# DocF/multispectral-object-detection

Measured on AMD Instinct MI355X. Metric: image-pairs/sec fwd, yolov5l+CFTx3 640×640 bs64, 1/2/4/8 GPU, higher is better.
Workload: dtype bf16; 1 GPU; cfg3 (yolov5l_fusion_transformerx3_FLIR_aligned) two-stream forward, 640x640, 64 pairs/GPU, BN folded, pre-NMS detections; pairs_per_gpu=64, image_size=640, parallelism=batch-shard x1, hip_graph=True, two_hip_streams=False, forwards_in_flight=3, streams_per_forward_in_flight=1, single_in_flight_streams=2

## Files before the change

### include/cft_hip.h

```cpp
#ifndef CFT_HIP_H
#define CFT_HIP_H

#ifdef __cplusplus
extern "C" {
#endif

#define CFT_ABI_VERSION 19

enum { CFT_BF16 = 0, CFT_F32 = 1, CFT_F16 = 2 };
enum { CFT_ACT_NONE = 0, CFT_ACT_SILU = 1, CFT_ACT_GELU = 2 };
enum {
  CFT_OK = 0,
  CFT_EINVAL = -1,
  CFT_ELAUNCH = -2,
  CFT_ENODEV = -3
};

int cft_abi_version(void);
int cft_device_check(void);
const char* cft_last_error(void);
int cft_clock_probe(void* out4_u64, int spin_us, int* wall_khz, void* stream);

int cft_conv2d(const void* x, const void* w, const float* bias, const void* res, void* y,
               int B, int H, int W, int cin, int ldx, int xoff,
// ... 158 lines not shown

int cft_gpt_upsample_add2(const float* tokens, const void* base0, int ldb0, int boff0, const void* base1, int ldb1, int boff1,
                          void* out0, int ldo0, int ooff0, void* out1, int ldo1, int ooff1, void* sum, int lds, int soff,
                          int B, int H, int W, int C, int dtype, void* stream);

int cft_gpt_tokenize_grid(const void* rgb, int ld_rgb, int off_rgb, const void* ir, int ld_ir, int off_ir,
                          const float* pos_emb, float* tokens, int B, int H, int W, int C, int va, int ha,
                          int dtype, void* stream);

int cft_attention_tokens(const void* qkv, void* out, int B, int T, int heads, int dk, int dkp,
                         int dtype, float attn_pdrop, unsigned long long seed, void* stream);

int cft_gpt_upsample_add_grid(const float* tokens, int s, const void* base, int ldb, int boff,
                              void* out, int ldo, int ooff, int B, int H, int W, int C, int va, int ha,
                              int dtype, void* stream);

int cft_gpt_upsample_add2_grid(const float* tokens, const void* base0, int ldb0, int boff0, const void* base1, int ldb1, int boff1,
                               void* out0, int ldo0, int ooff0, void* out1, int ldo1, int ooff1, void* sum, int lds, int soff,
                               int B, int H, int W, int C, int va, int ha, int dtype, void* stream);

int cft_detect_decode(const float* logits, int ldl, float* raw, float* pred, const float* anchors,
                      int B, int ny, int nx, int na, int no, float stride,
                      long row0, long total_rows, void* stream);

long cft_batchnorm_train_workspace(long M, int C);
int cft_batchnorm_train(const float* x, int ldx, int xoff, long M, int C,
                        const float* gamma, const float* beta, float* running_mean, float* running_var,
                        float momentum, float eps, const void* res, int ldr, int roff, int res_dtype,
                        void* y, int ldy, int yoff, int act, int out_dtype,
                        void* workspace, long workspace_bytes, void* stream);
int cft_dropout(void* x, long n, float p, unsigned long long seed, int dtype, void* stream);

int cft_nms(const float* pred, int B, int rows, int no, float conf_thres, float iou_thres,
            int agnostic, int multi_label, const unsigned char* class_allow, int max_det, int max_nms,
            void* scratch, long scratch_bytes, float* dets, int* counts, void* stream);

long cft_eval_match_workspace_bytes(int B, int nt);
int cft_eval_match(const float* dets, const int* counts, int B, int max_det, const float* targets, int nt, int img_h, int img_w,
                   const float* geom, const float* iouv_host, int niou, int single_cls, void* workspace, long workspace_bytes,
                   unsigned char* correct, unsigned short* tp_bits, float* conf, int* pcls, int* label_hist, int nc,
                   int* tcls, int* nl, void* stream);

long cft_eval_ap_workspace_bytes(long n, int nc);
int cft_eval_ap(const unsigned short* tp_bits, const float* conf, const int* pcls, long n, int niou, const int* label_hist, int nc,
                const double* px, const double* x, void* workspace, long workspace_bytes, double* out, void* stream);

// ... 80 lines not shown
```

### multispectral-object-detection_amd/_lib.py

```python
import ctypes
import os
import re
import subprocess

import torch

_HERE = os.path.dirname(os.path.abspath(__file__))
LIB_PATH = os.environ.get("CFT_HIP_LIB") or os.path.join(_HERE, "libcft_hip.so")
CSRC = os.path.join(_HERE, "csrc")
SOURCES = ("runtime.hip", "conv_gemm.hip", "conv_gemm_asm.hip", "focus_conv.hip", "bottleneck.hip", "pointwise.hip", "attention.hip", "attention_tokens.hip", "nms.hip", "train.hip", "metrics.hip", "confusion.hip", "loss.hip", "autoanchor.hip", "dataset.hip", "detect.hip", "optim.hip", "mosaic.hip", "augment.hip", "jpeg.hip", "jpeg_encode.hip")

HEADER = os.path.join(_HERE, "..", "include", "cft_hip.h")
HEADERS = ("cft_common.h", "conv_common.h", "focus_common.h", "bneck_common.h", "metrics_common.h", "resize_common.h", "conv_gemm_asm.inc")

_SCALARS = {"int": ctypes.c_int, "long": ctypes.c_long, "float": ctypes.c_float, "unsigned long long": ctypes.c_ulonglong}
_RETURNS = {"int": ctypes.c_int, "long": ctypes.c_long, "const char*": ctypes.c_char_p}
_TYPE_WORDS = frozenset("void char short int long float double signed unsigned const".split())


def parse_header(text):
    text = re.sub(r"/\*.*?\*/|//[^\n]*", " ", text, flags=re.S)
    consts = {k: int(v) for k, v in re.findall(r"(?:#define\s+|\b)(CFT_\w+)\s*=?\s*(-?\d+)\b", text)}
    text = re.sub(r"^\s*#.*$", "", text, flags=re.M)
    sigs = {}
    for ret, name, args in re.findall(r"([\w\s*]+?)\b(cft_\w+)\s*\(([^()]*)\)\s*;", text):
        ret = re.sub(r"\s*\*", "*", " ".join(ret.split()))
        if ret not in _RETURNS:
            raise ValueError(f"{name}: unknown return type '{ret}'")
        argtypes = []
        for arg in ([] if args.strip() in ("", "void") else args.split(",")):
            *kind, pname = [w for w in arg.split() if w != "const"] or [""]
            if "*" in arg:
                argtypes.append(ctypes.c_void_p)
            elif " ".join(kind) in _SCALARS and pname not in _TYPE_WORDS:
                argtypes.append(_SCALARS[" ".join(kind)])
            else:
# ... 73 lines not shown
```

### multispectral-object-detection_amd/csrc/conv_common.h

```cpp
#pragma once
#include "cft_common.h"
#include <stdlib.h>

struct ConvParams {
  const unsigned char* x;
  const unsigned char* w;
  const float* bias;
  const unsigned char* res;
  unsigned char* y;
  int H, W, Cin, ldx, xoff;
  int Ho, Wo, N, Kpad, K;
  int ldy, yoff, ldr, roff;
  int KS, stride, pad;
  int act, out_f32, res_f32;
  int M, tilesN;
  const unsigned char* w2;
  const float* bias2;
  int N2;
  unsigned char* y1;
  int ldy1, yoff1;
  int ksplit, ksteps;
  long x_bytes, w_bytes;
  uint32_t wo_mul, wo_sh, ho_mul, ho_sh;
};

__device__ __forceinline__ int fast_div(int n, uint32_t mul, uint32_t sh) {
  return mul ? (int)(__umulhi((uint32_t)n, mul) >> sh) : n;
}

static __device__ __attribute__((aligned(16))) uint32_t cft_zero_page[4] = {0u, 0u, 0u, 0u};
constexpr int CFT_ZERO_REGION_BYTES = 65536;
static __device__ __attribute__((aligned(128))) uint32_t cft_zero_region[CFT_ZERO_REGION_BYTES / 4];

typedef __attribute__((address_space(3))) void lds_void_t;
typedef const __attribute__((address_space(1))) void gbl_void_t;

template <typename TH, int WM, int WN, int ACT, bool OUT_F32>
__device__ __forceinline__ void conv_epilogue_impl(const ConvParams& p, f32x4_t (&acc)[WM / 16][WN / 16], unsigned char* smem,
                                                   int m0, int n0, int wm, int wn, int wave, int lane, const float (&bias_v)[WN / 16]) {
  constexpr int MT = WM / 16, NT = WN / 16;
  const int lrow = lane & 15, lgrp = lane >> 4;
  constexpr int SLD = WN + 4;
  float* stage = reinterpret_cast<float*>(smem) + wave * (16 * SLD);
  constexpr int VPRB = WN / 8;
  constexpr int VPL = (16 * VPRB + 63) / 64;
  constexpr int RDEPTH = (MT * VPL <= 6) ? MT : 2;
// ... 67 lines not shown
            Elem<TH>::unpack(rpre[i % RDEPTH][vi], rf);
#pragma unroll
            for (int e = 0; e < 8; ++e) v[e] += rf[e];
          } else if (p.res != nullptr) {
            const long ro = (long)m * p.ldr + p.roff + n;
            const float4 r0v = *reinterpret_cast<const float4*>(p.res + ro * 4);
            const float4 r1v = *reinterpret_cast<const float4*>(p.res + ro * 4 + 16);
            v[0] += r0v.x; v[1] += r0v.y; v[2] += r0v.z; v[3] += r0v.w;
            v[4] += r1v.x; v[5] += r1v.y; v[6] += r1v.z; v[7] += r1v.w;
          }
          *reinterpret_cast<gran_t*>(p.y + ((long)m * p.ldy + p.yoff + n) * 2) = Elem<TH>::pack(v);
        }
      }
      if (res_pre && i + RDEPTH < MT) CFT_RES_FETCH(i + RDEPTH)
    }
    __builtin_amdgcn_fence(__ATOMIC_RELEASE, "wavefront");
    __builtin_amdgcn_wave_barrier();
    __builtin_amdgcn_fence(__ATOMIC_ACQUIRE, "wavefront");
  }
}

#undef CFT_RES_FETCH

template <int WN>
__device__ __forceinline__ void conv_load_bias(const ConvParams& p, int n0, int wn, int lane, float (&bias_v)[WN / 16]) {
#pragma unroll
  for (int j = 0; j < WN / 16; ++j) {
    const int n = n0 + wn * WN + j * 16 + (lane & 15);
    bias_v[j] = (p.bias != nullptr && n < p.N) ? p.bias[n] : 0.0f;
  }
}

template <typename TH, int WM, int WN>
__device__ __forceinline__ void conv_epilogue(const ConvParams& p, f32x4_t (&acc)[WM / 16][WN / 16], unsigned char* smem,
                                              int m0, int n0, int wm, int wn, int wave, int lane, const float (&bias_v)[WN / 16]) {
  if (p.out_f32) {
    if (p.act == CFT_ACT_SILU) conv_epilogue_impl<TH, WM, WN, CFT_ACT_SILU, true>(p, acc, smem, m0, n0, wm, wn, wave, lane, bias_v);
    else if (p.act == CFT_ACT_GELU) conv_epilogue_impl<TH, WM, WN, CFT_ACT_GELU, true>(p, acc, smem, m0, n0, wm, wn, wave, lane, bias_v);
    else conv_epilogue_impl<TH, WM, WN, CFT_ACT_NONE, true>(p, acc, smem, m0, n0, wm, wn, wave, lane, bias_v);
  } else {
    if (p.act == CFT_ACT_SILU) conv_epilogue_impl<TH, WM, WN, CFT_ACT_SILU, false>(p, acc, smem, m0, n0, wm, wn, wave, lane, bias_v);
    else if (p.act == CFT_ACT_GELU) conv_epilogue_impl<TH, WM, WN, CFT_ACT_GELU, false>(p, acc, smem, m0, n0, wm, wn, wave, lane, bias_v);
    else conv_epilogue_impl<TH, WM, WN, CFT_ACT_NONE, false>(p, acc, smem, m0, n0, wm, wn, wave, lane, bias_v);
  }
}

// ... 11 lines not shown
```

### multispectral-object-detection_amd/csrc/conv_gemm.hip

```cpp
#include "conv_common.h"

template <typename T, int BM, int BN, int WGM, int WGN, bool GLDS, int ABLATE = 0, bool UNIK = false, bool CHAIN = false, bool CRES = false>
__global__ void __launch_bounds__(64 * WGM * WGN) conv_gemm_kernel(const ConvParams p) {
  constexpr int NTHR = 64 * WGM * WGN;
  constexpr int GE = Elem<T>::GE;
  constexpr int BK = 8 * GE;
  constexpr int RPP = NTHR / 8;
  constexpr int A_PER = BM / RPP, B_PER = (BN + RPP - 1) / RPP;
  constexpr int WM = BM / WGM, WN = BN / WGN, MT = WM / 16, NT = WN / 16;
  constexpr int A_BYTES = BM * 128, B_BYTES = BN * 128;
  constexpr int ES = (int)sizeof(T);
  static_assert(BM % RPP == 0 && BN % 8 == 0 && WM % 16 == 0 && WN % 16 == 0, "tile shape");
  extern __shared__ __attribute__((aligned(16))) unsigned char smem[];
  unsigned char* sA = smem;
  unsigned char* sB = smem + 2 * A_BYTES;

  const int nb = gridDim.x, bid = blockIdx.x;
  const int q = nb >> 3, r = nb & 7, xcd = bid & 7, slot = bid >> 3;
  const int logical = (xcd < r ? xcd * (q + 1) : r * (q + 1) + (xcd - r) * q) + slot;
  int ltile = logical, split = 0;
  if (p.ksplit > 1) {
    const int per = nb / p.ksplit;
    split = logical / per;
    ltile = logical - split * per;
  }
// ... 326 lines not shown
    p2.N = p.N2;
    p2.res = nullptr;
    conv_epilogue<TH, WM, WN>(p2, acc, smem, m0, 0, wm, wn, wave, lane, bias2_v);
    return;
  }
  if constexpr (ABLATE & 16) {
#pragma unroll
    for (int i = 0; i < MT; ++i)
#pragma unroll
      for (int j = 0; j < NT; ++j) asm volatile("" ::"v"(acc[i][j]));
    return;
  }
  if constexpr (ABLATE & 32) conv_load_bias<WN>(p, n0, wn, lane, bias_v);
  if (p.ksplit > 1) {
    ConvParams ps = p;
    ps.y = p.y + (long)split * p.M * p.ldy * 4;
    if (split != 0) {
#pragma unroll
      for (int j = 0; j < NT; ++j) bias_v[j] = 0.0f;
    }
    conv_epilogue_impl<typename Half16<T>::type, WM, WN, CFT_ACT_NONE, true>(ps, acc, smem, m0, n0, wm, wn, wave, lane, bias_v);
    return;
  }
  conv_epilogue<typename Half16<T>::type, WM, WN>(p, acc, smem, m0, n0, wm, wn, wave, lane, bias_v);
}

static void set_magic(int d, uint32_t& mul, uint32_t& sh) {
  if (d <= 1) { mul = 0; sh = 0; return; }
  int l = 0;
  while ((1L << l) < d) ++l;
  const unsigned long long k = 31ULL + l;
  mul = (uint32_t)(((1ULL << k) / (unsigned long long)d) + 1ULL);
  sh = (uint32_t)(k - 32);
}


thread_local int g_conv_variant = 0;
extern "C" int cft_set_conv_variant(int v) {
  const int old = g_conv_variant;
  g_conv_variant = v;
  return old;
}

int cft_set_conv_variant_peek() { return g_conv_variant; }

template <typename T, int BM, int BN, int WGM, int WGN, bool GLDS, int ABLATE = 0, bool UNIK = false, bool CHAIN = false, bool CRES = false>
static int launch_conv(const ConvParams& p, hipStream_t stream) {
  constexpr int smem_bytes = (CHAIN && BN / 64 > 2) ? (BN / 64) * BM * 128 + BN * 128 : 2 * (BM + BN) * 128;
  static_assert(!CHAIN || (BN / 64) * BM * 128 >= 2 * (BM + BN) * 128 || BN / 64 <= 2, "chained GEMM: LDS map");
  cft_allow_lds<&conv_gemm_kernel<T, BM, BN, WGM, WGN, GLDS, ABLATE, UNIK, CHAIN, CRES>>(smem_bytes);
  ConvParams q = p;
  const int tilesM = (p.M + BM - 1) / BM;
  q.tilesN = (p.N + BN - 1) / BN;
  if (q.ksplit < 1) q.ksplit = 1;
  if (!UNIK && q.ksplit > 1) {
    cft_set_error("conv_gemm_kernel: split-K needs the uniform-K-walk instantiation (this variant forces the generic address path)");
    return CFT_EINVAL;
  }
  hipLaunchKernelGGL((conv_gemm_kernel<T, BM, BN, WGM, WGN, GLDS, ABLATE, UNIK, CHAIN, CRES>), dim3(tilesM * q.tilesN * q.ksplit), dim3(64 * WGM * WGN), smem_bytes, stream, q);
  return cft_check_launch("conv_gemm_kernel");
}

template <typename T, int BM, int BN, int WGM, int WGN>
static int launch_auto(const ConvParams& p, hipStream_t stream) {
  constexpr int BK = 8 * Elem<T>::GE;
  const bool unik = g_conv_variant != 900 && p.Cin % BK == 0 && p.Kpad == p.K && 2L * p.Kpad * (long)sizeof(T) + 128 <= CFT_ZERO_REGION_BYTES;
  if (unik) return launch_conv<T, BM, BN, WGM, WGN, true, 0, true>(p, stream);
  return launch_conv<T, BM, BN, WGM, WGN, true>(p, stream);
}

#ifdef CFT_PROBES
template <typename T>
static bool ring_ok(const ConvParams& p) {
  return sizeof(T) == 2 && p.Cin % 64 == 0 && p.Kpad == p.K && p.KS <= 3 &&
         p.x_bytes + 2L * ((long)p.W + 1) * p.ldx < (1L << 31) && p.w_bytes < (1L << 31);
}

template <typename T, int ABLATE = 0>
static int launch_ring(const ConvParams& p, hipStream_t stream) {
  return conv_ring_launch(p, sizeof(T) != 2 ? CFT_F32 : (__is_same(T, f16_t) ? CFT_F16 : CFT_BF16), ABLATE, stream);
}
#endif

template <typename T>
static constexpr int dtype_code() { return sizeof(T) != 2 ? CFT_F32 : (__is_same(T, f16_t) ? CFT_F16 : CFT_BF16); }

template <typename T>
static int dispatch_conv(const ConvParams& p, hipStream_t stream) {
  switch (g_conv_variant) {
    case 96: case 961: case 962: case 963: case 964:
      if (conv_asm_ok(p, dtype_code<T>())) return conv_asm_launch(p, dtype_code<T>(), g_conv_variant == 96 ? 0 : g_conv_variant - 960, stream);
      break;
    case 1: return launch_conv<T, 128, 128, 2, 2, false>(p, stream);
    case 2: return launch_auto<T, 128, 128, 2, 2>(p, stream);
    case 4: return launch_auto<T, 128, 64, 2, 2>(p, stream);
    case 6: return launch_auto<T, 256, 64, 4, 2>(p, stream);
    case 7: return launch_auto<T, 64, 128, 2, 2>(p, stream);
    case 8: return launch_auto<T, 64, 64, 2, 2>(p, stream);
    case 23: return launch_auto<T, 128, 128, 2, 4>(p, stream);
    case 27: return launch_auto<T, 256, 256, 4, 4>(p, stream);
    case 30: return launch_auto<T, 512, 128, 8, 2>(p, stream);
    case 32: return launch_auto<T, 512, 64, 8, 2>(p, stream);
    case 33: return launch_auto<T, 256, 128, 4, 2>(p, stream);
    case 51: return launch_auto<T, 192, 128, 2, 4>(p, stream);
    case 60: return launch_auto<T, 128, 256, 4, 4>(p, stream);
    case 63: return launch_auto<T, 64, 128, 2, 4>(p, stream);
    case 70: return launch_auto<T, 256, 160, 8, 2>(p, stream);
    case 71: return launch_auto<T, 256, 160, 4, 2>(p, stream);
    case 72: return launch_auto<T, 128, 160, 4, 2>(p, stream);
    case 73: return launch_auto<T, 256, 80, 4, 1>(p, stream);
    case 74: return launch_auto<T, 256, 80, 8, 1>(p, stream);
// ... 65 lines not shown
  CFT_REQUIRE(cin % ge == 0 && ldx % ge == 0 && xoff % ge == 0, "cft_conv2d: input channels/ld/offset not granule aligned");
  CFT_REQUIRE(kpad % bk == 0 && kpad >= ksize * ksize * cin, "cft_conv2d: kpad must cover k*k*cin and be a multiple of the K step");
  CFT_REQUIRE(n % 8 == 0 && ldy % 8 == 0 && yoff % 8 == 0, "cft_conv2d: n/ldy/yoff must be multiples of 8");
  CFT_REQUIRE(res == nullptr || (ldr % 8 == 0 && roff % 8 == 0), "cft_conv2d: residual ld/offset must be multiples of 8");
  const int pad = ksize / 2;
  const int Ho = (H + 2 * pad - ksize) / stride + 1, Wo = (W + 2 * pad - ksize) / stride + 1;
  const long M = (long)B * Ho * Wo;
  CFT_REQUIRE(M < (1L << 31) && (long)B * H * W * ldx < (1L << 31) && M * ldy < (1L << 31),
              "cft_conv2d: tensor exceeds 2^31 elements (split the batch)");
  p.x = (const unsigned char*)x; p.w = (const unsigned char*)w; p.bias = bias;
  p.res = (const unsigned char*)res; p.y = (unsigned char*)y;
  p.H = H; p.W = W; p.Cin = cin; p.ldx = ldx; p.xoff = xoff;
  p.Ho = Ho; p.Wo = Wo; p.N = n; p.Kpad = kpad; p.K = ksize * ksize * cin;
  p.ldy = ldy; p.yoff = yoff; p.ldr = ldr; p.roff = roff;
  p.KS = ksize; p.stride = stride; p.pad = pad;
  p.act = act; p.out_f32 = out_dtype == CFT_F32; p.res_f32 = res_dtype == CFT_F32;
  p.M = (int)M; p.tilesN = 0;
  p.w2 = nullptr; p.bias2 = nullptr; p.N2 = 0;
  p.y1 = nullptr; p.ldy1 = 0; p.yoff1 = 0; p.ksplit = 1; p.ksteps = 0;
  p.x_bytes = (long)B * H * W * ldx * cft_elem_size(dtype);
  p.w_bytes = (long)n * kpad * cft_elem_size(dtype);
  set_magic(Wo, p.wo_mul, p.wo_sh);
  set_magic(Ho, p.ho_mul, p.ho_sh);
  return CFT_OK;
}

extern "C" int cft_conv2d(const void* x, const void* w, const float* bias, const void* res, void* y,
                          int B, int H, int W, int cin, int ldx, int xoff,
                          int n, int kpad, int ksize, int stride,
                          int ldy, int yoff, int ldr, int roff,
                          int act, int dtype, int out_dtype, int res_dtype, void* stream) {
  ConvParams p;
  const int rc = fill_conv_params(p, x, w, bias, res, y, B, H, W, cin, ldx, xoff, n, kpad, ksize, stride,
                                  ldy, yoff, ldr, roff, act, dtype, out_dtype, res_dtype);
  if (rc != CFT_OK) return rc;
  CFT_DISPATCH_DTYPE(dtype, T, return dispatch_conv<T>(p, as_stream(stream)));
  return CFT_EINVAL;
}

static bool chain_ok(const ConvParams& p, int n2, int dtype) {
  return (dtype == CFT_BF16 || dtype == CFT_F16) && (p.N == 128 || p.N == 256) && n2 >= 8 && n2 <= p.N && n2 % 8 == 0 && p.Cin % 64 == 0 && p.Kpad == p.K &&
         2L * p.Kpad * 2 + 128 <= CFT_ZERO_REGION_BYTES;
}

template <typename T>
static int dispatch_chain(const ConvParams& p, hipStream_t stream) {
  if constexpr (sizeof(T) == 2) {
    if (p.N == 128) return launch_conv<T, 192, 128, 2, 4, true, 0, true, true>(p, stream);
    if (g_conv_variant != 97 && conv_asm_chain_ok(p, dtype_code<T>())) return conv_asm_chain_launch(p, dtype_code<T>(), stream);
    if (p.y1 != nullptr) return launch_conv<T, 256, 256, 4, 4, true, 0, true, true, true>(p, stream);
    return launch_conv<T, 256, 256, 4, 4, true, 0, true, true>(p, stream);
  } else return CFT_EINVAL;
}

extern "C" int cft_conv2d_chain(const void* x, const void* w1, const float* bias1, const void* w2, const float* bias2, void* y,
                                int B, int H, int W, int cin, int ldx, int xoff,
                                int n1, int kpad1, int ksize, int stride, int n2,
                                int ldy, int yoff, int act2, int dtype, void* stream) {
  CFT_REQUIRE(w2 != nullptr, "cft_conv2d_chain: null pointer");
  ConvParams p;
  const int rc = fill_conv_params(p, x, w1, bias1, nullptr, y, B, H, W, cin, ldx, xoff, n1, kpad1, ksize, stride,
// ... 60 lines not shown
```

### multispectral-object-detection_amd/csrc/pointwise.hip

```cpp
#include "cft_common.h"
#include "resize_common.h"

static inline int grid_for(long work, int block) {
  long g = (work + block - 1) / block;
  const long cap = 256L * 16;
  return (int)(g < 1 ? 1 : (g > cap ? cap : g));
}

template <typename T>
__global__ void __launch_bounds__(256) focus_s2d_kernel(const float* __restrict__ in, unsigned char* __restrict__ out,
                                                        int B, int H, int W) {
  const int Ho = H >> 1, Wo = W >> 1;
  const long total = (long)B * Ho * Wo;
  for (long idx = (long)blockIdx.x * blockDim.x + threadIdx.x; idx < total; idx += (long)gridDim.x * blockDim.x) {
    const int x = (int)(idx % Wo);
    const long t = idx / Wo;
    const int y = (int)(t % Ho);
    const int b = (int)(t / Ho);
    float v[16];
#pragma unroll
    for (int c = 0; c < 3; ++c) {
      const float* base = in + (((long)b * 3 + c) * H + 2 * y) * W + 2 * x;
      const float2 top = *reinterpret_cast<const float2*>(base);
      const float2 bot = *reinterpret_cast<const float2*>(base + W);
// ... 527 lines not shown
      const int x = idx / gpc, cgl = idx - x * gpc;
      const long cb = (long)(c0 + cgl * GE) * sizeof(T);
      float fx = ((float)x + 0.5f) * sx - 0.5f; fx = fx < 0.f ? 0.f : fx;
      const int x0 = (int)fx, x1 = x0 + (x0 < ha - 1 ? 1 : 0);
      const float lx = fx - (float)x0, hx = 1.f - lx;
      const long pix = rowpix + x;
      const float* r0 = R + x0 * CW + cgl * GE;
      const float* r1 = R + x1 * CW + cgl * GE;
      float v0[GE];
      if (DUAL || base0 != nullptr) {
        Elem<T>::unpack(*reinterpret_cast<const gran_t*>(base0 + pix * ldb0_b + boff0_b + cb), v0);
      } else {
#pragma unroll
        for (int e = 0; e < GE; ++e) v0[e] = 0.f;
      }
      if constexpr (DUAL) {
        float v1[GE];
        Elem<T>::unpack(*reinterpret_cast<const gran_t*>(base1 + pix * ldb1_b + boff1_b + cb), v1);
#pragma unroll
        for (int e = 0; e < GE; ++e) {
          v0[e] += hx * r0[e] + lx * r1[e];
          v1[e] += hx * r0[ha * CW + e] + lx * r1[ha * CW + e];
        }
        *reinterpret_cast<gran_t*>(out0 + pix * ldo0_b + ooff0_b + cb) = Elem<T>::pack(v0);
        *reinterpret_cast<gran_t*>(out1 + pix * ldo1_b + ooff1_b + cb) = Elem<T>::pack(v1);
        if (sum != nullptr) {
#pragma unroll
          for (int e = 0; e < GE; ++e) v0[e] += v1[e];
          *reinterpret_cast<gran_t*>(sum + pix * lds_b + soff_b + cb) = Elem<T>::pack(v0);
        }
      } else {
#pragma unroll
        for (int e = 0; e < GE; ++e) v0[e] += hx * r0[e] + lx * r1[e];
        *reinterpret_cast<gran_t*>(out0 + pix * ldo0_b + ooff0_b + cb) = Elem<T>::pack(v0);
      }
    }
  }
}

static inline int gpt_upsample_grid_chunk(int C, int ha, int ns) {
  int cw = (16 * 1024) / (ns * ha);
  cw -= cw % 8;
  return C < cw ? C : cw;
}

template <bool DUAL, int VA, int HA>
static int gpt_upsample_launch(const char* who, const float* tokens, int s, ChanRef base0, ChanRef base1, ChanRef out0, ChanRef out1, ChanRef sum,
                               int B, int H, int W, int C, int va, int ha, int dtype, void* stream) {
// ... 13 lines not shown
  const size_t smem = (size_t)NS * ha * cw * sizeof(float);
  CFT_DISPATCH_DTYPE(dtype, T, {
    if constexpr (DUAL && VA != 0) cft_allow_lds<&gpt_upsample_kernel<T, DUAL, VA, HA>>(128 * 1024);
    hipLaunchKernelGGL((gpt_upsample_kernel<T, DUAL, VA, HA>), dim3(B * H), dim3(256), smem, as_stream(stream), tokens, s,
                       base0.ptr(), base0.ld * es, base0.off * es, base1.ptr(), base1.ld * es, base1.off * es,
                       out0.ptr(), out0.ld * es, out0.off * es, out1.ptr(), out1.ld * es, out1.off * es,
                       sum.ptr(), sum.ld * es, sum.off * es, B, H, W, C, va, ha, cw);
  });
  return cft_check_launch("gpt_upsample_kernel");
}

extern "C" int cft_gpt_upsample_add(const float* tokens, int s, const void* base, int ldb, int boff,
                                    void* out, int ldo, int ooff, int B, int H, int W, int C,
                                    int dtype, void* stream) {
  CFT_REQUIRE(tokens && out, "cft_gpt_upsample_add: null pointer");
  CFT_REQUIRE(cft_is_dtype(dtype), "cft_gpt_upsample_add: bad dtype");
  CFT_REQUIRE(s == 0 || s == 1, "cft_gpt_upsample_add: stream index must be 0 or 1");
  return gpt_upsample_launch<false, 8, 8>("cft_gpt_upsample_add", tokens, s, {base, ldb, boff}, {}, {out, ldo, ooff}, {}, {}, B, H, W, C, 8, 8, dtype, stream);
}

extern "C" int cft_gpt_upsample_add2(const float* tokens, const void* base0, int ldb0, int boff0, const void* base1, int ldb1, int boff1,
                                     void* out0, int ldo0, int ooff0, void* out1, int ldo1, int ooff1, void* sum, int lds, int soff,
                                     int B, int H, int W, int C, int dtype, void* stream) {
  CFT_REQUIRE(tokens && base0 && base1 && out0 && out1, "cft_gpt_upsample_add2: null pointer");
  CFT_REQUIRE(cft_is_dtype(dtype), "cft_gpt_upsample_add2: bad dtype");
  return gpt_upsample_launch<true, 8, 8>("cft_gpt_upsample_add2", tokens, 0, {base0, ldb0, boff0}, {base1, ldb1, boff1}, {out0, ldo0, ooff0},
                                         {out1, ldo1, ooff1}, {sum, lds, soff}, B, H, W, C, 8, 8, dtype, stream);
}

extern "C" int cft_gpt_upsample_add_grid(const float* tokens, int s, const void* base, int ldb, int boff,
                                         void* out, int ldo, int ooff, int B, int H, int W, int C, int va, int ha,
                                         int dtype, void* stream) {
  CFT_REQUIRE(tokens && out, "cft_gpt_upsample_add_grid: null pointer");
  CFT_REQUIRE(cft_is_dtype(dtype), "cft_gpt_upsample_add_grid: bad dtype");
  CFT_REQUIRE(s == 0 || s == 1, "cft_gpt_upsample_add_grid: stream index must be 0 or 1");
  CFT_REQUIRE(cft_grid_ok(va, ha), "cft_gpt_upsample_add_grid: " CFT_GRID_RULE);
  return gpt_upsample_launch<false, 0, 0>("cft_gpt_upsample_add_grid", tokens, s, {base, ldb, boff}, {}, {out, ldo, ooff}, {}, {}, B, H, W, C, va, ha, dtype, stream);
}

extern "C" int cft_gpt_upsample_add2_grid(const float* tokens, const void* base0, int ldb0, int boff0, const void* base1, int ldb1, int boff1,
                                          void* out0, int ldo0, int ooff0, void* out1, int ldo1, int ooff1, void* sum, int lds, int soff,
                                          int B, int H, int W, int C, int va, int ha, int dtype, void* stream) {
  CFT_REQUIRE(tokens && base0 && base1 && out0 && out1, "cft_gpt_upsample_add2_grid: null pointer");
  CFT_REQUIRE(cft_is_dtype(dtype), "cft_gpt_upsample_add2_grid: bad dtype");
  CFT_REQUIRE(cft_grid_ok(va, ha), "cft_gpt_upsample_add2_grid: " CFT_GRID_RULE);
  return gpt_upsample_launch<true, 0, 0>("cft_gpt_upsample_add2_grid", tokens, 0, {base0, ldb0, boff0}, {base1, ldb1, boff1}, {out0, ldo0, ooff0},
                                         {out1, ldo1, ooff1}, {sum, lds, soff}, B, H, W, C, va, ha, dtype, stream);
}

__global__ void __launch_bounds__(256) detect_decode_kernel(const float* __restrict__ logits, int ldl, float* __restrict__ raw,
                                                            float* __restrict__ pred, const float* __restrict__ anchors,
                                                            int B, int ny, int nx, int na, int no, float stride,
                                                            long row0, long total_rows) {
  const long total = (long)B * na * ny * nx * no;
  for (long idx = (long)blockIdx.x * blockDim.x + threadIdx.x; idx < total; idx += (long)gridDim.x * blockDim.x) {
    const int o = (int)(idx % no);
    long t = idx / no;
    const int x = (int)(t % nx); t /= nx;
    const int y = (int)(t % ny); t /= ny;
    const int a = (int)(t % na);
    const int b = (int)(t / na);
    const float v = logits[(((long)b * ny + y) * nx + x) * ldl + a * no + o];
    raw[idx] = v;
    const float sg = 1.0f / (1.0f + __expf(-v));
    float r;
    if (o == 0) r = (sg * 2.0f - 0.5f + (float)x) * stride;
    else if (o == 1) r = (sg * 2.0f - 0.5f + (float)y) * stride;
    else if (o < 4) { const float w = sg * 2.0f; r = w * w * anchors[a * 2 + (o - 2)]; }
    else r = sg;
    pred[((long)b * total_rows + row0 + ((long)a * ny + y) * nx + x) * no + o] = r;
  }
}

extern "C" int cft_detect_decode(const float* logits, int ldl, float* raw, float* pred, const float* anchors,
                                 int B, int ny, int nx, int na, int no, float stride,
                                 long row0, long total_rows, void* stream) {
  CFT_REQUIRE(logits && raw && pred && anchors, "cft_detect_decode: null pointer");
  CFT_REQUIRE(B > 0 && ny > 0 && nx > 0 && na > 0 && no >= 5 && ldl >= na * no, "cft_detect_decode: bad shape");
  CFT_REQUIRE(row0 >= 0 && row0 + (long)na * ny * nx <= total_rows, "cft_detect_decode: rows out of range");
  const long total = (long)B * na * ny * nx * no;
  hipLaunchKernelGGL(detect_decode_kernel, dim3(grid_for(total, 256)), dim3(256), 0, as_stream(stream), logits, ldl, raw, pred, anchors,
                     B, ny, nx, na, no, stride, row0, total_rows);
  return cft_check_launch("detect_decode_kernel");
}

__global__ void __launch_bounds__(256) letterbox_u8_kernel(const unsigned char* __restrict__ src, int sh, int sw, long src_row_stride,
                                                           unsigned char* __restrict__ dst, int dh, int dw, long dsy, long dsx, long dsc, int flip,
                                                           int rh, int rw, int top, int left, int c0, int c1, int c2) {
  const long total = (long)dh * dw;
  const double scale_x = cft_linear_scale(rw, sw), scale_y = cft_linear_scale(rh, sh);
  const bool resize = rh != sh || rw != sw;
  for (long idx = (long)blockIdx.x * blockDim.x + threadIdx.x; idx < total; idx += (long)gridDim.x * blockDim.x) {
    const int y = (int)(idx / dw), x = (int)(idx - (long)y * dw);
// ... 37 lines not shown
```

### multispectral-object-detection_amd/models/common.py

```python
import math
from collections import namedtuple

import torch
import torch.nn as nn

from .. import ops
from ..ops import ACT_GELU, ACT_NONE, ACT_SILU

BN_EPS = 1e-3


def autopad(k, p=None):
    if p is None:
        p = k // 2 if isinstance(k, int) else [x // 2 for x in k]
    return p


class _Pending:

    def materialize(self):
        raise NotImplementedError


class PendingBilinear(_Pending):
# ... 21 lines not shown

    @property
    def shape(self):
        B, C, H, W = self.x.shape
        return torch.Size((B, C, H << self.up, W << self.up))


class PendingConv(_Pending):

    def __init__(self, conv, x):
        self.conv, self.x = conv, x

    def materialize(self):
        return self.conv(self.x)

    @property
    def shape(self):
        B, _, H, W = self.x.shape
        return torch.Size((B, self.conv.conv.out_channels, *ops.conv_out_size(H, W, self.conv.conv.kernel_size[0], self.conv.conv.stride[0])))


def resolve(x):
    return x.materialize() if isinstance(x, _Pending) else x


def _cache_key(module, dtype, device):
    vers = tuple((int(p.data_ptr()), int(p._version)) for p in module.parameters()) \
        + tuple((int(b.data_ptr()), int(b._version)) for b in module.buffers())
    return (dtype, str(device), vers)


def invalidate_packed(root):
    for m in root.modules():
        m.__dict__.pop("_cft_cache", None)
        m.__dict__.pop("_cft_cache_train", None)
        m.__dict__.pop("_plan_cache", None)
        if "_graphs" in m.__dict__:
            m.__dict__["_graphs"].clear()
        m.__dict__.pop("_wlist", None)


class _Packed(nn.Module):

    def _packed(self, dtype, device, train=False):
        key = (train,) + _cache_key(self, dtype, device)
        slot = "_cft_cache_train" if train else "_cft_cache"
# ... 677 lines not shown
```

### multispectral-object-detection_amd/models/layer_graph.py

```python
from functools import cached_property

import torch.nn as nn

from .common import GPT, SPP, Add, Add2, C3, Concat, Conv, Focus


def graph_key(layers):
    return tuple(id(m) for m in layers)


class LayerGraph:
    def __init__(self, layers):
        self.layers = layers = list(layers)
        self.key = graph_key(layers)
        self.image = []
        self.multi = []
        self.sources = []
        for i, m in enumerate(layers):
            f = m.f
            self.image.append(1 if f == -4 else 0 if i == 0 else None)
            self.multi.append(not isinstance(f, int))
            self.sources.append([] if self.image[i] is not None else [i + j if j < 0 else j for j in ([f] if isinstance(f, int) else f)])
        self._segments = {}

    def inputs(self, i, prev, y):
        vals = [prev if j == i - 1 else y[j] for j in self.sources[i]]
        return vals if self.multi[i] else vals[0]

    @cached_property
    def readers(self):
        readers = {}
        for j, srcs in enumerate(self.sources):
            for s in srcs:
                readers.setdefault(s, set()).add(j)
        return readers

    @cached_property
    def lanes(self):
        lanes = []
        for i, m in enumerate(self.layers):
            if self.image[i] is not None:
                lane = self.image[i]
            elif not self.multi[i] or isinstance(m, Add2):
                lane = lanes[self.sources[i][0]]
            else:
                lane = 0
# ... 84 lines not shown
```

### multispectral-object-detection_amd/ops.py

```python
from dataclasses import dataclass
from typing import Optional

import torch

from . import _lib
from ._lib import ACT_GELU, ACT_NONE, ACT_SILU, CFT_BF16, CFT_F16, CFT_F32


COMPUTE_DTYPES = (torch.bfloat16, torch.float16, torch.float32)


def _dt(dtype):
    if dtype == torch.bfloat16:
        return CFT_BF16
    if dtype == torch.float16:
        return CFT_F16
    if dtype == torch.float32:
        return CFT_F32
    raise TypeError(f"compute dtype must be torch.bfloat16, torch.float16 or torch.float32, got {dtype}")


def _stream():
    return torch.cuda.current_stream().cuda_stream

# ... 520 lines not shown
                         f"got {tuple(tokens.shape)} {tokens.dtype}")
    B, T, C = tokens.shape
    out = new_nhwc(B, H, W, C, dtype, tokens.device)
    bp, ldb = None, 0
    if base is not None:
        base, ldb = as_nhwc(base)
        if tuple(base.shape) != (B, C, H, W) or base.dtype != dtype:
            raise ValueError("gpt_upsample_add: base shape/dtype mismatch")
        bp = base.data_ptr()
    lib = _lib.load()
    fn, label, grid_args = _grid_entry(lib, "cft_gpt_upsample_add", va, ha)
    st = _timed("cft_upsample_add", 0.0, (2.0 if bp else 1.0) * B * H * W * C * out.element_size(),
                lambda: fn(tokens.data_ptr(), s, bp, ldb, 0, out.data_ptr(), C, 0, B, H, W, C, *grid_args, _dt(dtype), _stream()))
    _lib.check(st, label)
    return out


def gpt_dual_tokens_ok(tokens, grid=None):
    va, ha = (int(g) for g in token_grid(tokens, grid))
    return (isinstance(tokens, torch.Tensor) and tokens.is_cuda and tokens.dim() == 3 and tokens.shape[1] == 2 * va * ha
            and tokens.dtype == torch.float32 and tokens.is_contiguous() and tokens.shape[2] % 4 == 0 and tokens.data_ptr() % 16 == 0)


def gpt_upsample_add_dual(tokens, base0, base1, H, W, dtype, sum_out=None, want_sum=True, grid=None):
    _require_cuda(tokens, "gpt_upsample_add_dual")
    grid = token_grid(tokens, grid)
    va, ha = _grid(grid)
    if not gpt_dual_tokens_ok(tokens, grid):
        raise ValueError(f"gpt_upsample_add_dual: tokens must be a contiguous, 16-byte aligned fp32 [B, {2 * va * ha}, C] tensor (C % 4 == 0), "
                         f"got {tuple(tokens.shape)} {tokens.dtype}")
    B, T, C = tokens.shape
    base0, ldb0 = as_nhwc(base0)
    base1, ldb1 = as_nhwc(base1)
    for bse in (base0, base1):
        if tuple(bse.shape) != (B, C, H, W) or bse.dtype != dtype:
            raise ValueError("gpt_upsample_add_dual: base shape/dtype mismatch")
    out0 = new_nhwc(B, H, W, C, dtype, tokens.device)
    out1 = new_nhwc(B, H, W, C, dtype, tokens.device)
    sp, lds = None, 0
    if want_sum:
        if sum_out is None:
            sum_out = new_nhwc(B, H, W, C, dtype, tokens.device)
        if tuple(sum_out.shape) != (B, C, H, W) or sum_out.dtype != dtype:
            raise ValueError("gpt_upsample_add_dual: sum_out shape/dtype mismatch")
        lds = _view_ld(sum_out, "gpt_upsample_add_dual sum")
        sp = sum_out.data_ptr()
    else:
        sum_out = None
    lib = _lib.load()
    fn, label, grid_args = _grid_entry(lib, "cft_gpt_upsample_add2", va, ha)
    st = _timed("cft_upsample_add", 0.0, (5.0 if want_sum else 4.0) * B * H * W * C * out0.element_size(),
                lambda: fn(tokens.data_ptr(), base0.data_ptr(), ldb0, 0, base1.data_ptr(), ldb1, 0, out0.data_ptr(), C, 0, out1.data_ptr(), C, 0,
                           sp, lds, 0, B, H, W, C, *grid_args, _dt(dtype), _stream()))
    _lib.check(st, label)
    return out0, out1, sum_out


def detect_decode(logits, raw, pred, anchors_px, na, no, stride, row0):
    B, ldl, ny, nx = logits.shape
    st = _lib.load().cft_detect_decode(logits.data_ptr(), ldl, raw.data_ptr(), pred.data_ptr(), anchors_px.data_ptr(),
                                       B, ny, nx, na, no, float(stride), row0, pred.shape[1], _stream())
    _lib.check(st, "cft_detect_decode")


def pair_batch_u8(desc_dev, desc_host, out, color=114):
    _require_cuda(out, "pair_batch_u8")
    _require_cuda(desc_dev, "pair_batch_u8")
    B = out.shape[0]
    if out.dtype != torch.uint8 or out.dim() != 4 or out.shape[1] != 6 or not out.is_contiguous():
        raise ValueError(f"pair_batch_u8: out must be a contiguous uint8 [B, 6, H, W] tensor, got {out.dtype} {tuple(out.shape)}")
    for t, what in ((desc_dev, "desc_dev"), (desc_host, "desc_host")):
        if t.dtype != torch.uint8 or tuple(t.shape) != (B, _lib._consts["CFT_PAIR_DESC_BYTES"]) or not t.is_contiguous():
            raise ValueError(f"pair_batch_u8: {what} must be a contiguous uint8 [{B}, {_lib._consts['CFT_PAIR_DESC_BYTES']}] tensor")
    if desc_host.is_cuda:
        raise ValueError("pair_batch_u8: desc_host must be a host tensor")
    st = _lib.load().cft_pair_batch_u8(desc_dev.data_ptr(), desc_host.data_ptr(), B, out.data_ptr(), out.shape[2], out.shape[3], int(color), _stream())
    _lib.check(st, "cft_pair_batch_u8")
    return out


def augment_batch_u8(desc_dev, desc_host, luts, out):
    _require_cuda(out, "augment_batch_u8")
    _require_cuda(desc_dev, "augment_batch_u8")
    _require_cuda(luts, "augment_batch_u8")
    B, nbytes = out.shape[0], _lib._consts["CFT_AUG_DESC_BYTES"]
# ... 225 lines not shown
```

Baseline: 3660 image-pairs/sec.

## Fuse detect head 1x1 conv with anchor decode in GEMM epilogue

Adds a decode epilogue to the conv GEMM kernel, so the detect head's 1x1 conv writes raw and decoded predictions directly. This removes the fp32 logits round trip and the separate decode kernel launch. A DetectLaunch wrapper routes Detect layers to the fused path when rows are large enough and the output width fits one 64-wide tile. Separately, gpt_upsample_add_dual can now skip writing the per-stream outputs when only the sum is needed, although no caller in this change uses that option yet. The epilogue stages results through LDS and scatters them with divisions per element, which may be slower than the plain epilogue. The fused path also bypasses the asm and variant conv dispatch.

```diff
diff --git a/include/cft_hip.h b/include/cft_hip.h
--- a/include/cft_hip.h
+++ b/include/cft_hip.h
@@ -204,6 +204,11 @@
 int cft_detect_decode(const float* logits, int ldl, float* raw, float* pred, const float* anchors,
                       int B, int ny, int nx, int na, int no, float stride,
                       long row0, long total_rows, void* stream);
+
+int cft_detect_conv(const void* x, const void* w, const float* bias, float* raw, float* pred, const float* anchors,
+                    int B, int H, int W, int cin, int ldx, int xoff, int n, int kpad,
+                    int na, int no, float stride, long row0, long total_rows, int dtype, void* stream);
+int cft_detect_conv_ok(int n, int na, int no);
 
 long cft_batchnorm_train_workspace(long M, int C);
 int cft_batchnorm_train(const float* x, int ldx, int xoff, long M, int C,
diff --git a/multispectral-object-detection_amd/_lib.py b/multispectral-object-detection_amd/_lib.py
--- a/multispectral-object-detection_amd/_lib.py
+++ b/multispectral-object-detection_amd/_lib.py
@@ -11,7 +11,7 @@
 SOURCES = ("runtime.hip", "conv_gemm.hip", "conv_gemm_asm.hip", "focus_conv.hip", "bottleneck.hip", "pointwise.hip", "attention.hip", "attention_tokens.hip", "nms.hip", "train.hip", "metrics.hip", "confusion.hip", "loss.hip", "autoanchor.hip", "dataset.hip", "detect.hip", "optim.hip", "mosaic.hip", "augment.hip", "jpeg.hip", "jpeg_encode.hip")
 
 HEADER = os.path.join(_HERE, "..", "include", "cft_hip.h")
-HEADERS = ("cft_common.h", "conv_common.h", "focus_common.h", "bneck_common.h", "metrics_common.h", "resize_common.h", "conv_gemm_asm.inc")
+HEADERS = ("cft_common.h", "conv_common.h", "focus_common.h", "bneck_common.h", "metrics_common.h", "resize_common.h", "detect_common.h", "conv_gemm_asm.inc")
 
 _SCALARS = {"int": ctypes.c_int, "long": ctypes.c_long, "float": ctypes.c_float, "unsigned long long": ctypes.c_ulonglong}
 _RETURNS = {"int": ctypes.c_int, "long": ctypes.c_long, "const char*": ctypes.c_char_p}
diff --git a/multispectral-object-detection_amd/csrc/conv_common.h b/multispectral-object-detection_amd/csrc/conv_common.h
--- a/multispectral-object-detection_amd/csrc/conv_common.h
+++ b/multispectral-object-detection_amd/csrc/conv_common.h
@@ -1,5 +1,6 @@
 #pragma once
 #include "cft_common.h"
+#include "detect_common.h"
 #include <stdlib.h>
 
 struct ConvParams {
@@ -22,6 +23,13 @@
   int ksplit, ksteps;
   long x_bytes, w_bytes;
   uint32_t wo_mul, wo_sh, ho_mul, ho_sh;
+  float* dec_raw;
+  float* dec_pred;
+  const float* dec_anchors;
+  int dec_na, dec_no;
+  float dec_stride;
+  long dec_row0, dec_rows;
+  uint32_t no_mul, no_sh;
 };
 
 __device__ __forceinline__ int fast_div(int n, uint32_t mul, uint32_t sh) {
@@ -135,6 +143,51 @@
 
 #undef CFT_RES_FETCH
 
+template <int WM, int WN>
+__device__ __forceinline__ void conv_epilogue_decode(const ConvParams& p, f32x4_t (&acc)[WM / 16][WN / 16], unsigned char* smem,
+                                                     int m0, int n0, int wm, int wn, int wave, int lane, const float (&bias_v)[WN / 16]) {
+  constexpr int MT = WM / 16, NT = WN / 16;
+  const int lrow = lane & 15, lgrp = lane >> 4;
+  constexpr int SLD = WN + 4;
+  float* stage = reinterpret_cast<float*>(smem) + wave * (16 * SLD);
+  const int nbase = n0 + wn * WN;
+  const int nval = p.dec_na * p.dec_no;
+  if (nbase >= nval) return;
+  const int no = p.dec_no;
+  const int a_lo = fast_div(nbase, p.no_mul, p.no_sh);
+  const int a_hi = fast_div((nbase + WN < nval ? nbase + WN : nval) - 1, p.no_mul, p.no_sh);
+  const long hw = (long)p.Ho * p.Wo;
+#pragma unroll
+  for (int i = 0; i < MT; ++i) {
+#pragma unroll
+    for (int j = 0; j < NT; ++j)
+#pragma unroll
+      for (int e = 0; e < 4; ++e)
+        stage[(lgrp * 4 + e) * SLD + j * 16 + lrow] = apply_act<CFT_ACT_NONE>(acc[i][j][e] + bias_v[j]);
+    __builtin_amdgcn_fence(__ATOMIC_RELEASE, "wavefront");
+    __builtin_amdgcn_wave_barrier();
+    __builtin_amdgcn_fence(__ATOMIC_ACQUIRE, "wavefront");
+    const int mbase = m0 + wm * WM + i * 16;
+    for (int a = a_lo; a <= a_hi; ++a) {
+      for (int idx = lane; idx < 16 * no; idx += 64) {
+        const int row = fast_div(idx, p.no_mul, p.no_sh), o = idx - row * no;
+        const int m = mbase + row, col = a * no + o - nbase;
+        if (m < p.M && col >= 0 && col < WN) {
+          const float v = stage[row * SLD + col];
+          const int t = fast_div(m, p.wo_mul, p.wo_sh), x = m - t * p.Wo;
+          const int b = fast_div(t, p.ho_mul, p.ho_sh), y = t - b * p.Ho;
+          const long cell = (long)a * hw + (m - b * hw);
+          p.dec_raw[((long)b * p.dec_na * hw + cell) * no + o] = v;
+          p.dec_pred[((long)b * p.dec_rows + p.dec_row0 + cell) * no + o] = detect_decode_value(v, o, x, y, a, p.dec_anchors, p.dec_stride);
+        }
+      }
+    }
+    __builtin_amdgcn_fence(__ATOMIC_RELEASE, "wavefront");
+    __builtin_amdgcn_wave_barrier();
+    __builtin_amdgcn_fence(__ATOMIC_ACQUIRE, "wavefront");
+  }
+}
+
 template <int WN>
 __device__ __forceinline__ void conv_load_bias(const ConvParams& p, int n0, int wn, int lane, float (&bias_v)[WN / 16]) {
 #pragma unroll
diff --git a/multispectral-object-detection_amd/csrc/conv_gemm.hip b/multispectral-object-detection_amd/csrc/conv_gemm.hip
--- a/multispectral-object-detection_amd/csrc/conv_gemm.hip
+++ b/multispectral-object-detection_amd/csrc/conv_gemm.hip
@@ -1,6 +1,6 @@
 #include "conv_common.h"
 
-template <typename T, int BM, int BN, int WGM, int WGN, bool GLDS, int ABLATE = 0, bool UNIK = false, bool CHAIN = false, bool CRES = false>
+template <typename T, int BM, int BN, int WGM, int WGN, bool GLDS, int ABLATE = 0, bool UNIK = false, bool CHAIN = false, bool CRES = false, bool DEC = false>
 __global__ void __launch_bounds__(64 * WGM * WGN) conv_gemm_kernel(const ConvParams p) {
   constexpr int NTHR = 64 * WGM * WGN;
   constexpr int GE = Elem<T>::GE;
@@ -373,6 +373,11 @@
     conv_epilogue_impl<typename Half16<T>::type, WM, WN, CFT_ACT_NONE, true>(ps, acc, smem, m0, n0, wm, wn, wave, lane, bias_v);
     return;
   }
+  if constexpr (DEC) {
+    static_assert(BN <= 64 && ABLATE == 0 && !CHAIN, "decode epilogue: narrow plain tiles");
+    conv_epilogue_decode<WM, WN>(p, acc, smem, m0, n0, wm, wn, wave, lane, bias_v);
+    return;
+  }
   conv_epilogue<typename Half16<T>::type, WM, WN>(p, acc, smem, m0, n0, wm, wn, wave, lane, bias_v);
 }
 
@@ -395,11 +400,11 @@
 
 int cft_set_conv_variant_peek() { return g_conv_variant; }
 
-template <typename T, int BM, int BN, int WGM, int WGN, bool GLDS, int ABLATE = 0, bool UNIK = false, bool CHAIN = false, bool CRES = false>
+template <typename T, int BM, int BN, int WGM, int WGN, bool GLDS, int ABLATE = 0, bool UNIK = false, bool CHAIN = false, bool CRES = false, bool DEC = false>
 static int launch_conv(const ConvParams& p, hipStream_t stream) {
   constexpr int smem_bytes = (CHAIN && BN / 64 > 2) ? (BN / 64) * BM * 128 + BN * 128 : 2 * (BM + BN) * 128;
   static_assert(!CHAIN || (BN / 64) * BM * 128 >= 2 * (BM + BN) * 128 || BN / 64 <= 2, "chained GEMM: LDS map");
-  cft_allow_lds<&conv_gemm_kernel<T, BM, BN, WGM, WGN, GLDS, ABLATE, UNIK, CHAIN, CRES>>(smem_bytes);
+  cft_allow_lds<&conv_gemm_kernel<T, BM, BN, WGM, WGN, GLDS, ABLATE, UNIK, CHAIN, CRES, DEC>>(smem_bytes);
   ConvParams q = p;
   const int tilesM = (p.M + BM - 1) / BM;
   q.tilesN = (p.N + BN - 1) / BN;
@@ -408,16 +413,16 @@
     cft_set_error("conv_gemm_kernel: split-K needs the uniform-K-walk instantiation (this variant forces the generic address path)");
     return CFT_EINVAL;
   }
-  hipLaunchKernelGGL((conv_gemm_kernel<T, BM, BN, WGM, WGN, GLDS, ABLATE, UNIK, CHAIN, CRES>), dim3(tilesM * q.tilesN * q.ksplit), dim3(64 * WGM * WGN), smem_bytes, stream, q);
+  hipLaunchKernelGGL((conv_gemm_kernel<T, BM, BN, WGM, WGN, GLDS, ABLATE, UNIK, CHAIN, CRES, DEC>), dim3(tilesM * q.tilesN * q.ksplit), dim3(64 * WGM * WGN), smem_bytes, stream, q);
   return cft_check_launch("conv_gemm_kernel");
 }
 
-template <typename T, int BM, int BN, int WGM, int WGN>
+template <typename T, int BM, int BN, int WGM, int WGN, bool DEC = false>
 static int launch_auto(const ConvParams& p, hipStream_t stream) {
   constexpr int BK = 8 * Elem<T>::GE;
   const bool unik = g_conv_variant != 900 && p.Cin % BK == 0 && p.Kpad == p.K && 2L * p.Kpad * (long)sizeof(T) + 128 <= CFT_ZERO_REGION_BYTES;
-  if (unik) return launch_conv<T, BM, BN, WGM, WGN, true, 0, true>(p, stream);
-  return launch_conv<T, BM, BN, WGM, WGN, true>(p, stream);
+  if (unik) return launch_conv<T, BM, BN, WGM, WGN, true, 0, true, false, false, DEC>(p, stream);
+  return launch_conv<T, BM, BN, WGM, WGN, true, 0, false, false, false, DEC>(p, stream);
 }
 
 #ifdef CFT_PROBES
@@ -438,6 +443,13 @@
 
 template <typename T>
 static int dispatch_conv(const ConvParams& p, hipStream_t stream) {
+  if (p.dec_raw != nullptr) {
+    auto wgs = [&](int bm) { return (long)((p.M + bm - 1) / bm); };
+    if (p.N <= 32) return wgs(128) >= 512 ? launch_auto<T, 128, 32, 4, 1, true>(p, stream) : launch_auto<T, 64, 32, 2, 1, true>(p, stream);
+    if (wgs(256) >= 192) return launch_auto<T, 256, 64, 4, 2, true>(p, stream);
+    if (wgs(128) >= 192) return launch_auto<T, 128, 64, 2, 2, true>(p, stream);
+    return launch_auto<T, 64, 64, 2, 2, true>(p, stream);
+  }
   switch (g_conv_variant) {
     case 96: case 961: case 962: case 963: case 964:
       if (conv_asm_ok(p, dtype_code<T>())) return conv_asm_launch(p, dtype_code<T>(), g_conv_variant == 96 ? 0 : g_conv_variant - 960, stream);
@@ -549,6 +561,8 @@
   p.w_bytes = (long)n * kpad * cft_elem_size(dtype);
   set_magic(Wo, p.wo_mul, p.wo_sh);
   set_magic(Ho, p.ho_mul, p.ho_sh);
+  p.dec_raw = nullptr; p.dec_pred = nullptr; p.dec_anchors = nullptr; p.dec_na = 0; p.dec_no = 0; p.dec_stride = 0.f;
+  p.dec_row0 = 0; p.dec_rows = 0; p.no_mul = 0; p.no_sh = 0;
   return CFT_OK;
 }
 
@@ -564,6 +578,27 @@
   CFT_DISPATCH_DTYPE(dtype, T, return dispatch_conv<T>(p, as_stream(stream)));
   return CFT_EINVAL;
 }
+
+extern "C" int cft_detect_conv(const void* x, const void* w, const float* bias, float* raw, float* pred, const float* anchors,
+                               int B, int H, int W, int cin, int ldx, int xoff, int n, int kpad,
+                               int na, int no, float stride, long row0, long total_rows, int dtype, void* stream) {
+  CFT_REQUIRE(raw && pred && anchors, "cft_detect_conv: null pointer");
+  CFT_REQUIRE(na > 0 && no >= 5 && (long)na * no <= n && n <= 64, "cft_detect_conv: na * no must fit n, and n one 64-wide tile (ask cft_detect_conv_ok)");
+  CFT_REQUIRE(H > 0 && W > 0 && row0 >= 0 && row0 + (long)na * H * W <= total_rows, "cft_detect_conv: rows out of range");
+  ConvParams p;
+  static float unused_y;
+  const int rc = fill_conv_params(p, x, w, bias, nullptr, &unused_y, B, H, W, cin, ldx, xoff, n, kpad, 1, 1,
+                                  n, 0, 0, 0, CFT_ACT_NONE, dtype, CFT_F32, dtype);
+  if (rc != CFT_OK) return rc;
+  p.y = nullptr;
+  p.dec_raw = raw; p.dec_pred = pred; p.dec_anchors = anchors; p.dec_na = na; p.dec_no = no; p.dec_stride = stride;
+  p.dec_row0 = row0; p.dec_rows = total_rows;
+  set_magic(no, p.no_mul, p.no_sh);
+  CFT_DISPATCH_DTYPE(dtype, T, return dispatch_conv<T>(p, as_stream(stream)));
+  return CFT_EINVAL;
+}
+
+extern "C" int cft_detect_conv_ok(int n, int na, int no) { return (na > 0 && no >= 5 && (long)na * no <= n && n % 8 == 0 && n <= 64) ? 1 : 0; }
 
 static bool chain_ok(const ConvParams& p, int n2, int dtype) {
   return (dtype == CFT_BF16 || dtype == CFT_F16) && (p.N == 128 || p.N == 256) && n2 >= 8 && n2 <= p.N && n2 % 8 == 0 && p.Cin % 64 == 0 && p.Kpad == p.K &&
diff --git a/multispectral-object-detection_amd/csrc/detect_common.h b/multispectral-object-detection_amd/csrc/detect_common.h
--- /dev/null
+++ b/multispectral-object-detection_amd/csrc/detect_common.h
@@ -0,0 +1,11 @@
+#pragma once
+
+__device__ __forceinline__ float detect_decode_value(float v, int o, int x, int y, int a, const float* __restrict__ anchors, float stride) {
+  const float sg = 1.0f / (1.0f + __expf(-v));
+  float r;
+  if (o == 0) r = (sg * 2.0f - 0.5f + (float)x) * stride;
+  else if (o == 1) r = (sg * 2.0f - 0.5f + (float)y) * stride;
+  else if (o < 4) { const float w = sg * 2.0f; r = w * w * anchors[a * 2 + (o - 2)]; }
+  else r = sg;
+  return r;
+}
diff --git a/multispectral-object-detection_amd/csrc/pointwise.hip b/multispectral-object-detection_amd/csrc/pointwise.hip
--- a/multispectral-object-detection_amd/csrc/pointwise.hip
+++ b/multispectral-object-detection_amd/csrc/pointwise.hip
@@ -1,5 +1,6 @@
 #include "cft_common.h"
 #include "resize_common.h"
+#include "detect_common.h"
 
 static inline int grid_for(long work, int block) {
   long g = (work + block - 1) / block;
@@ -573,8 +574,8 @@
           v0[e] += hx * r0[e] + lx * r1[e];
           v1[e] += hx * r0[ha * CW + e] + lx * r1[ha * CW + e];
         }
-        *reinterpret_cast<gran_t*>(out0 + pix * ldo0_b + ooff0_b + cb) = Elem<T>::pack(v0);
-        *reinterpret_cast<gran_t*>(out1 + pix * ldo1_b + ooff1_b + cb) = Elem<T>::pack(v1);
+        if (out0 != nullptr) *reinterpret_cast<gran_t*>(out0 + pix * ldo0_b + ooff0_b + cb) = Elem<T>::pack(v0);
+        if (out1 != nullptr) *reinterpret_cast<gran_t*>(out1 + pix * ldo1_b + ooff1_b + cb) = Elem<T>::pack(v1);
         if (sum != nullptr) {
 #pragma unroll
           for (int e = 0; e < GE; ++e) v0[e] += v1[e];
@@ -634,7 +635,7 @@
 extern "C" int cft_gpt_upsample_add2(const float* tokens, const void* base0, int ldb0, int boff0, const void* base1, int ldb1, int boff1,
                                      void* out0, int ldo0, int ooff0, void* out1, int ldo1, int ooff1, void* sum, int lds, int soff,
                                      int B, int H, int W, int C, int dtype, void* stream) {
-  CFT_REQUIRE(tokens && base0 && base1 && out0 && out1, "cft_gpt_upsample_add2: null pointer");
+  CFT_REQUIRE(tokens && base0 && base1 && ((out0 && out1) || sum), "cft_gpt_upsample_add2: null pointer (out0 / out1 may be NULL only when sum is not)");
   CFT_REQUIRE(cft_is_dtype(dtype), "cft_gpt_upsample_add2: bad dtype");
   return gpt_upsample_launch<true, 8, 8>("cft_gpt_upsample_add2", tokens, 0, {base0, ldb0, boff0}, {base1, ldb1, boff1}, {out0, ldo0, ooff0},
                                          {out1, ldo1, ooff1}, {sum, lds, soff}, B, H, W, C, 8, 8, dtype, stream);
@@ -653,7 +654,7 @@
 extern "C" int cft_gpt_upsample_add2_grid(const float* tokens, const void* base0, int ldb0, int boff0, const void* base1, int ldb1, int boff1,
                                           void* out0, int ldo0, int ooff0, void* out1, int ldo1, int ooff1, void* sum, int lds, int soff,
                                           int B, int H, int W, int C, int va, int ha, int dtype, void* stream) {
-  CFT_REQUIRE(tokens && base0 && base1 && out0 && out1, "cft_gpt_upsample_add2_grid: null pointer");
+  CFT_REQUIRE(tokens && base0 && base1 && ((out0 && out1) || sum), "cft_gpt_upsample_add2_grid: null pointer (out0 / out1 may be NULL only when sum is not)");
   CFT_REQUIRE(cft_is_dtype(dtype), "cft_gpt_upsample_add2_grid: bad dtype");
   CFT_REQUIRE(cft_grid_ok(va, ha), "cft_gpt_upsample_add2_grid: " CFT_GRID_RULE);
   return gpt_upsample_launch<true, 0, 0>("cft_gpt_upsample_add2_grid", tokens, 0, {base0, ldb0, boff0}, {base1, ldb1, boff1}, {out0, ldo0, ooff0},
@@ -674,13 +675,7 @@
     const int b = (int)(t / na);
     const float v = logits[(((long)b * ny + y) * nx + x) * ldl + a * no + o];
     raw[idx] = v;
-    const float sg = 1.0f / (1.0f + __expf(-v));
-    float r;
-    if (o == 0) r = (sg * 2.0f - 0.5f + (float)x) * stride;
-    else if (o == 1) r = (sg * 2.0f - 0.5f + (float)y) * stride;
-    else if (o < 4) { const float w = sg * 2.0f; r = w * w * anchors[a * 2 + (o - 2)]; }
-    else r = sg;
-    pred[((long)b * total_rows + row0 + ((long)a * ny + y) * nx + x) * no + o] = r;
+    pred[((long)b * total_rows + row0 + ((long)a * ny + y) * nx + x) * no + o] = detect_decode_value(v, o, x, y, a, anchors, stride);
   }
 }
 
diff --git a/multispectral-object-detection_amd/models/common.py b/multispectral-object-detection_amd/models/common.py
--- a/multispectral-object-detection_amd/models/common.py
+++ b/multispectral-object-detection_amd/models/common.py
@@ -67,6 +67,40 @@
 
 def resolve(x):
     return x.materialize() if isinstance(x, _Pending) else x
+
+
+class DetectLaunch:
+    fuse_decode = True
+
+    def __init__(self, detect):
+        self.__dict__["detect"] = detect
+
+    def __getattr__(self, name):
+        return getattr(self.__dict__["detect"], name)
+
+    def __call__(self, x):
+        m = self.detect
+        if m.training or m.export or not self.fuse_decode:
+            return m(x)
+        x = [resolve(t) for t in x]
+        packed, anchors_px = m._packed(x[0].dtype, x[0].device)
+        B = x[0].shape[0]
+        fused = [t.is_cuda and B * t.shape[2] * t.shape[3] >= ops.HEAD_PASS_MIN_ROWS and ops.detect_conv_ok(pk, m.na, m.no) for t, pk in zip(x, packed)]
+        if not any(fused):
+            return m(x)
+        rows = [m.na * t.shape[2] * t.shape[3] for t in x]
+        pred = torch.empty((B, sum(rows), m.no), dtype=torch.float32, device=x[0].device)
+        raws, row0 = [], 0
+        for i, t in enumerate(x):
+            raw = torch.empty((B, m.na, t.shape[2], t.shape[3], m.no), dtype=torch.float32, device=t.device)
+            if fused[i]:
+                ops.detect_conv(t, packed[i], raw, pred, anchors_px[i], m.na, m.no, float(m.stride[i]), row0)
+            else:
+                logits = ops.conv2d(t, packed[i], ACT_NONE, out_dtype=torch.float32)
+                ops.detect_decode(logits, raw, pred, anchors_px[i], m.na, m.no, float(m.stride[i]), row0)
+            raws.append(raw)
+            row0 += rows[i]
+        return pred, raws
 
 
 def _cache_key(module, dtype, device):
diff --git a/multispectral-object-detection_amd/models/layer_graph.py b/multispectral-object-detection_amd/models/layer_graph.py
--- a/multispectral-object-detection_amd/models/layer_graph.py
+++ b/multispectral-object-detection_amd/models/layer_graph.py
@@ -2,7 +2,7 @@
 
 import torch.nn as nn
 
-from .common import GPT, SPP, Add, Add2, C3, Concat, Conv, Focus
+from .common import GPT, SPP, Add, Add2, C3, Concat, Conv, DetectLaunch, Focus
 
 
 def graph_key(layers):
@@ -22,6 +22,8 @@
             self.multi.append(not isinstance(f, int))
             self.sources.append([] if self.image[i] is not None else [i + j if j < 0 else j for j in ([f] if isinstance(f, int) else f)])
         self._segments = {}
+        from .yolo_test import Detect
+        self.layers = [DetectLaunch(m) if isinstance(m, Detect) else m for m in layers]
 
     def inputs(self, i, prev, y):
         vals = [prev if j == i - 1 else y[j] for j in self.sources[i]]
diff --git a/multispectral-object-detection_amd/ops.py b/multispectral-object-detection_amd/ops.py
--- a/multispectral-object-detection_amd/ops.py
+++ b/multispectral-object-detection_amd/ops.py
@@ -566,8 +566,10 @@
             and tokens.dtype == torch.float32 and tokens.is_contiguous() and tokens.shape[2] % 4 == 0 and tokens.data_ptr() % 16 == 0)
 
 
-def gpt_upsample_add_dual(tokens, base0, base1, H, W, dtype, sum_out=None, want_sum=True, grid=None):
+def gpt_upsample_add_dual(tokens, base0, base1, H, W, dtype, sum_out=None, want_sum=True, grid=None, want0=True, want1=True):
     _require_cuda(tokens, "gpt_upsample_add_dual")
+    if not want_sum and not (want0 and want1):
+        raise ValueError("gpt_upsample_add_dual: a map can be left out only when the sum is wanted")
     grid = token_grid(tokens, grid)
     va, ha = _grid(grid)
     if not gpt_dual_tokens_ok(tokens, grid):
@@ -579,8 +581,9 @@
     for bse in (base0, base1):
         if tuple(bse.shape) != (B, C, H, W) or bse.dtype != dtype:
             raise ValueError("gpt_upsample_add_dual: base shape/dtype mismatch")
-    out0 = new_nhwc(B, H, W, C, dtype, tokens.device)
-    out1 = new_nhwc(B, H, W, C, dtype, tokens.device)
+    out0 = new_nhwc(B, H, W, C, dtype, tokens.device) if want0 else None
+    out1 = new_nhwc(B, H, W, C, dtype, tokens.device) if want1 else None
+    p0, p1 = (None if o is None else o.data_ptr() for o in (out0, out1))
     sp, lds = None, 0
     if want_sum:
         if sum_out is None:
@@ -593,8 +596,8 @@
         sum_out = None
     lib = _lib.load()
     fn, label, grid_args = _grid_entry(lib, "cft_gpt_upsample_add2", va, ha)
-    st = _timed("cft_upsample_add", 0.0, (5.0 if want_sum else 4.0) * B * H * W * C * out0.element_size(),
-                lambda: fn(tokens.data_ptr(), base0.data_ptr(), ldb0, 0, base1.data_ptr(), ldb1, 0, out0.data_ptr(), C, 0, out1.data_ptr(), C, 0,
+    st = _timed("cft_upsample_add", 0.0, (2.0 + bool(want0) + bool(want1) + bool(want_sum)) * B * H * W * C * base0.element_size(),
+                lambda: fn(tokens.data_ptr(), base0.data_ptr(), ldb0, 0, base1.data_ptr(), ldb1, 0, p0, C, 0, p1, C, 0,
                            sp, lds, 0, B, H, W, C, *grid_args, _dt(dtype), _stream()))
     _lib.check(st, label)
     return out0, out1, sum_out
@@ -605,6 +608,32 @@
     st = _lib.load().cft_detect_decode(logits.data_ptr(), ldl, raw.data_ptr(), pred.data_ptr(), anchors_px.data_ptr(),
                                        B, ny, nx, na, no, float(stride), row0, pred.shape[1], _stream())
     _lib.check(st, "cft_detect_decode")
+
+
+HEAD_PASS_MIN_ROWS = 192 * 64
+
+
+def detect_conv_ok(pk, na, no):
+    return pk.k == 1 and pk.s == 1 and bool(_lib.load().cft_detect_conv_ok(pk.n, na, no))
+
+
+def detect_conv(x, pk, raw, pred, anchors_px, na, no, stride, row0):
+    _require_cuda(x, "detect_conv")
+    x, ldx = as_nhwc(x)
+    B, C, ny, nx = x.shape
+    if C != pk.cin:
+        raise ValueError(f"detect_conv: input has {C} channels, packed weight expects {pk.cin}")
+    if tuple(raw.shape) != (B, na, ny, nx, no) or tuple(pred.shape[::2]) != (B, no) or not (raw.is_contiguous() and pred.is_contiguous()) \
+            or raw.dtype != torch.float32 or pred.dtype != torch.float32:
+        raise ValueError("detect_conv: raw must be a contiguous fp32 [B, na, ny, nx, no] tensor and pred a contiguous fp32 [B, rows, no] one")
+    lib = _lib.load()
+    es = x.element_size()
+    abytes = B * ny * nx * pk.cin * es + 2 * B * ny * nx * na * no * 4 + pk.w.numel() * es
+    st = _timed(f"conv_k1s1_n{pk.n}_K{pk.kpad}_decode",B * ny * nx * pk.flops_per_row, abytes,
+                lambda: lib.cft_detect_conv(x.data_ptr(), pk.w.data_ptr(), _bias_ptr(pk), raw.data_ptr(), pred.data_ptr(), anchors_px.data_ptr(),
+                                            B, ny, nx, pk.cin, ldx, 0, pk.n, pk.kpad, na, no, float(stride), row0, pred.shape[1], _dt(x.dtype),
+                                            _stream()))
+    _lib.check(st, "cft_detect_conv")
 
 
 def pair_batch_u8(desc_dev, desc_host, out, color=114):
```

After: 3656 image-pairs/sec, median of 2. No clear change (-0.1%).
